# Yuki-11/CSBSR

Hardware: AMD Instinct MI355X
Metric: training imgs/s (448->1792 x4, PSPNet) (higher is better)
Workload: dtype fp16 storage / fp32 accumulate (detector forward: split fp16 hi+lo); 1 GPU; CSBSR KBPN x4 + PSPNet, beta=0.3, joint phase (iter 40000), per-GPU batch 8, LR 448x448 -> HR 1792x1792, fwd+loss+bwd+Adam; batch resident in HBM (H2D outside `value`, timed beside it as with_h2d_inside_step); full-size synthetic crack images degraded on the device; global_batch=8, micro_batch=8, parallelism=dp1

## Files before the change

csbsr_amd/_lib.py:

```python
import ctypes as C
import os
from collections import namedtuple

import torch

_HERE = os.path.dirname(os.path.abspath(__file__))
LIB_PATH = os.environ.get("CSBSR_LIB") or os.path.join(_HERE, "libcsbsr_hip.so")

ACT_NONE, ACT_RELU, ACT_LRELU, ACT_PRELU, ACT_SIGMOID = 0, 1, 2, 3, 4
RES_NONE, RES_ADD, RES_SUB, RES_MUL, RES_FMA = 0, 1, 2, 3, 4
STAT_NONE, STAT_BN, STAT_SAMPLE_SUM = 0, 1, 2

i32, i64, f32, vp = C.c_int32, C.c_int64, C.c_float, C.c_void_p


class Seg(C.Structure):
    _fields_ = [("ptr", vp), ("sn", i64), ("sy", i64), ("sx", i64), ("c", i32), ("creal", i32)]


class ConvDesc(C.Structure):
    _fields_ = [("inp", Seg * 2), ("N", i32), ("H", i32), ("W", i32), ("OH", i32), ("OW", i32),
                ("transposed", i32), ("KH", i32), ("KW", i32), ("stride", i32), ("pad", i32), ("dil", i32),
                ("wt", vp), ("cout", i32), ("coutp", i32),
                ("out16", vp), ("o_sn", i64), ("o_sy", i64), ("o_sx", i64),
# ... 73 lines not shown
    "csbsr_maxpool3x3s2_bwd_split": (i32, [vp, i64, i64, vp, i64, i64, vp, vp, i32, i32, i32, i32, vp]),
    "csbsr_adaptive_avgpool_fwd_split": (i32, [vp, i64, i64, vp, i64, i64, i32, i32, i32, i32, i32, i32, vp]),
    "csbsr_sum_act_split": (i32, [i64, i32, i32, vp, vp, vp, vp, i64, i64, i32, vp]),
    "csbsr_weighted_pool_fwd_split": (i32, [vp, i64, i64, vp, vp, i32, i64, i32, vp]),
    "csbsr_bilinear_fwd_split": (i32, [vp, i64, i64, vp, i64, i64, i32, i32, i32, i32, i32, i32, i32, vp, vp]),
    "csbsr_unpack_wgrad": (i32, [vp, vp] + [i32] * 9 + [f32, i32, i32, vp]),
    "csbsr_wgrad_splits": (i32, [i32, i32, i64]),
    "csbsr_wgrad_splits_desc": (i32, [vp]),
    "csbsr_epilogue_backward": (i32, [C.POINTER(EpiBwdDesc), vp]),
    "csbsr_set_reduction_scratch": (i32, [vp, i64]),
    "csbsr_axpby": (i32, [i64, i32, vp, i64, f32, vp, i64, f32, vp, i64, vp]),
    "csbsr_fill_f16": (i32, [vp, i64, i32, i64, f32, vp]),
    "csbsr_sum_act": (i32, [i64, i32, i32, vp, vp, vp, i64, i32, vp]),
    "csbsr_weighted_pool_fwd": (i32, [vp, i64, vp, vp, i32, i64, i32, vp]),
    "csbsr_weighted_pool_bwd": (i32, [vp, i64, vp, vp, vp, i64, vp, i32, i64, i32, vp]),
    "csbsr_nchw32_to_nhwc16": (i32, [vp, vp, i32, i32, i32, i32, i32, i64, vp, vp, vp]),
    "csbsr_nhwc16_to_nchw32": (i32, [vp, i64, vp, i32, i32, i32, i32, f32, f32, vp]),
    "csbsr_plane_reduce": (i32, [vp, vp, i32, i64, vp, vp]),
    "csbsr_channel_mean_sub": (i32, [vp, i64, i64, i64, i32, i32, i32, i32, i32, vp, vp]),
    "csbsr_thin_tp_backward_slabs": (i32, [i32, i32]),
    "csbsr_conv_thin_dact_eligible": (i32, [vp]),
    "csbsr_conv_split_fused_eligible": (i32, [C.POINTER(ConvDesc)]),
    "csbsr_thin_tp_backward": (i32, [vp, i64, i64, i64, vp, i64, i64, i64, vp, i32, i32, i32, i32, vp, i32, i32, i32, vp, i64, i64, i64, vp, vp, vp]),
    "csbsr_round_weights": (i32, [vp, vp, vp, i32, i32, i32, i32, i32, vp]),
    "csbsr_dc_bias": (i32, [vp, i32, i32, vp, i64, i32, vp, i64, i32, vp, i32, vp, vp]),
    "csbsr_instnorm_bwd": (i32, [vp, i64, vp, vp, vp, vp, i32, i32, i32, i64, vp, vp]),
    "csbsr_border_class_fill": (i32, [vp, vp, i64, i32, i32, i32, i32, vp]),
    "csbsr_border_class_fill_masked": (i32, [vp, vp, i64, vp, i64, C.c_float, i32, i32, i32, i32, vp]),
    "csbsr_border_class_sums": (i32, [vp, i64, vp, i32, i32, i32, i32, vp]),
    "csbsr_border_class_sums_prelu": (i32, [vp, i64, vp, i64, vp, vp, i32, i32, i32, i32, vp]),
    "csbsr_ring_class_sums": (i32, [vp, i64, vp, i32, i32, i32, i32, vp]),
    "csbsr_bn_finalize": (i32, [vp, i64, i32, i32, f32, f32, vp, vp, vp, vp, vp]),
    "csbsr_bn_apply": (i32, [C.POINTER(BnDesc), vp]),
    "csbsr_bn_backward": (i32, [C.POINTER(BnDesc), vp]),
    "csbsr_maxpool3x3s2_fwd": (i32, [vp, vp, i32, i32, i32, i32, vp]),
    "csbsr_maxpool3x3s2_bwd": (i32, [vp, vp, vp, vp, i32, i32, i32, i32, vp]),
    "csbsr_adaptive_avgpool_fwd": (i32, [vp, i64, vp, i32, i32, i32, i32, i32, i32, vp]),
    "csbsr_adaptive_avgpool_bwd": (i32, [vp, vp, i64, i32, i32, i32, i32, i32, i32, i32, vp]),
    "csbsr_bilinear_fwd": (i32, [vp, i64, vp, i64, i32, i32, i32, i32, i32, i32, i32, vp, vp]),
    "csbsr_bilinear_bwd": (i32, [vp, i64, vp, i64, i32, i32, i32, i32, i32, i32, i32, i32, vp, vp]),
    "csbsr_bilinear32_fwd": (i32, [vp, vp, i32, i32, i32, i32, i32, i32, vp]),
    "csbsr_bilinear32_bwd": (i32, [vp, vp, i32, i32, i32, i32, i32, i32, vp]),
    "csbsr_bicubic_up_add": (i32, [vp, vp, i32, i32, i32, i32, vp]),
    "csbsr_aa_bicubic_up": (i32, [vp, vp, i32, i32, i32, i32, i32, i32, vp]),
    "csbsr_aa_bicubic_down_fwd": (i32, [vp, vp, i32, i32, i32, i32, i32, vp]),
    "csbsr_aa_bicubic_down_bwd": (i32, [vp, vp, i32, i32, i32, i32, i32, i32, vp]),
    "csbsr_area_down_fwd": (i32, [vp, vp, i32, i32, i32, i32, vp]),
    "csbsr_area_down_bwd": (i32, [vp, vp, i32, i32, i32, i32, i32, vp]),
    "csbsr_blur_fwd": (i32, [vp, vp, i32, i32, i32, i32, i32, i32, vp, vp, vp, i64, vp]),
    "csbsr_blur_bwd_input": (i32, [vp, vp, vp, i32, i32, i32, i32, i32, i32, i32, vp]),
    "csbsr_blur_bwd_kernel": (i32, [vp, vp, vp, i32, i32, i32, i32, i32, i32, vp]),
    "csbsr_sdf": (i32, [vp, vp, vp, i32, i32, i32, vp]),
# ... 98 lines not shown
```

csbsr_amd/csrc/elementwise.hip:

```cpp
#include <cstdlib>
#include "common.h"

static inline int grid_for(long work, int block = 256, int cap = 8192) {
  long b = (work + block - 1) / block;
  if (b < 1) b = 1;
  return (int)(b > cap ? cap : b);
}
#define ST(s) reinterpret_cast<hipStream_t>(s)

__device__ __forceinline__ void ld_split(const half_t* p, long lo, float (&v)[8]) {
  const h8 a = *reinterpret_cast<const h8*>(p);
#pragma unroll
  for (int e = 0; e < 8; ++e) v[e] = (float)a[e];
  if (lo) {
    const h8 b = *reinterpret_cast<const h8*>(p + lo);
#pragma unroll
    for (int e = 0; e < 8; ++e) v[e] += (float)b[e];
  }
}
__device__ __forceinline__ void st_split(half_t* p, long lo, const float (&v)[8]) {
  h8 a, b;
#pragma unroll
  for (int e = 0; e < 8; ++e) { a[e] = (half_t)v[e]; b[e] = (half_t)(v[e] - (float)a[e]); }
  *reinterpret_cast<h8*>(p) = a;
// ... 1746 lines not shown
}
__global__ void bcs_edges_finish_kernel(const float* part, float* sums, int N, int c) {
  const int i = blockIdx.x * blockDim.x + threadIdx.x;
  if (i >= N * 4 * 3 * c) return;
  const int ch = i % c; int r = i / c;
  const int k = r % 3; r /= 3;
  const int edge = r % 4; const int n = r / 4;
  if (edge >= 2 && k > 0) return;
  const int base_cls = edge == 0 ? 8 : (edge == 1 ? 4 : (edge == 2 ? 2 : 1));
  const int cls = base_cls + (k == 1 ? 2 : (k == 2 ? 1 : 0));
  float t = 0.f;
  for (int seg = 0; seg < BCS_SEG; ++seg) t += part[((((long)n * 4 + edge) * BCS_SEG + seg) * 3 + k) * c + ch];
  sums[((long)n * 16 + cls) * c + ch] += t;
}
__global__ void bcs_fixup_kernel(float* sums, int N, int c) {
  const int i = blockIdx.x * blockDim.x + threadIdx.x;
  if (i >= N * c) return;
  const int n = i / c, ch = i % c;
  float* s_ = sums + (long)n * 16 * c + ch;
  float border = 0.f;
  for (int k = 1; k < 16; ++k) border += s_[(long)k * c];
  s_[0] -= border;
}
static int border_class_sums_impl(const void* x, int64_t ld, float* sums, int32_t N, int32_t H, int32_t W, int32_t c, const void* t, int64_t t_ld,
                                  float* negdot, csbsr_stream_t s) {
  CSBSR_CHECK(x && sums && c % 8 == 0, "border_class_sums: bad args");
  CSBSR_CHECK(!t || (negdot && H >= 3 && W >= 3 && (long)H * W >= 1024), "border_class_sums_prelu: maps of >= 1024 pixels, negdot required");
  if (H >= 3 && W >= 3 && (long)H * W >= 1024) {
    const long hw = (long)H * W;
    int chunks = (int)((hw + 511) / 512);
    if (chunks > 2048) chunks = 2048;
    const long n_tot = (long)N * chunks * c, n_edge = (long)N * 4 * BCS_SEG * 3 * c;
    float* part = csbsr_red_scratch(n_tot + n_edge + (t ? n_tot : 0));
    CSBSR_NEED_SCRATCH(part, "border_class_sums");
    if (t) {
      float* part2 = part + n_tot + n_edge;
      hipLaunchKernelGGL(bcs_total_kernel<true>, dim3(N * chunks), dim3(256), 0, ST(s), (const half_t*)x, (long)ld, sums, hw, c / 8, chunks, part,
                         (const half_t*)t, (long)t_ld, part2);
      if (csbsr_sum_partials_batched(part2, chunks, c, c, negdot, N, (long)c, ST(s))) return 1;
    } else {
      hipLaunchKernelGGL(bcs_total_kernel<false>, dim3(N * chunks), dim3(256), 0, ST(s), (const half_t*)x, (long)ld, sums, hw, c / 8, chunks, part,
                         (const half_t*)nullptr, 0l, (float*)nullptr);
    }
    if (csbsr_sum_partials_batched(part, chunks, c, c, sums, N, 16l * c, ST(s))) return 1;
    float* epart = part + n_tot;
    hipLaunchKernelGGL(bcs_edges_kernel, dim3(N * 4 * ((c / 8 + 31) / 32) * BCS_SEG), dim3(256), 0, ST(s), (const half_t*)x, (long)ld, epart, H, W, c / 8);
    hipLaunchKernelGGL(bcs_edges_finish_kernel, dim3((N * 12 * c + 255) / 256), dim3(256), 0, ST(s), (const float*)epart, sums, N, c);
    hipLaunchKernelGGL(bcs_fixup_kernel, dim3((N * c + 255) / 256), dim3(256), 0, ST(s), sums, N, c);
    CSBSR_LAUNCH_CHECK("csbsr_border_class_sums");
    return 0;
  }
  hipLaunchKernelGGL(border_class_sums_small_kernel, dim3(N), dim3(256), 0, ST(s), (const half_t*)x, (long)ld, sums, H, W, c / 8);
  CSBSR_LAUNCH_CHECK("csbsr_border_class_sums");
  return 0;
}
extern "C" int csbsr_border_class_sums(const void* x, int64_t ld, float* sums, int32_t N, int32_t H, int32_t W, int32_t c, csbsr_stream_t s) {
  return border_class_sums_impl(x, ld, sums, N, H, W, c, nullptr, 0, nullptr, s);
}
extern "C" int csbsr_border_class_sums_prelu(const void* x, int64_t ld, const void* t, int64_t t_ld, float* sums, float* negdot, int32_t N, int32_t H,
                                             int32_t W, int32_t c, csbsr_stream_t s) {
  CSBSR_CHECK(t && negdot, "border_class_sums_prelu: null pointer");
  return border_class_sums_impl(x, ld, sums, N, H, W, c, t, t_ld, negdot, s);
}

__global__ __launch_bounds__(256) void rcs_lines_kernel(const half_t* x, long ld, float* part, int H, int W, int c8) {
  __shared__ float sbin[8][5][32][8];
  const int groups = (c8 + 31) / 32;
  int b = blockIdx.x;
  const int seg = b % BCS_SEG; b /= BCS_SEG;
  const int g = b % groups; b /= groups;
  const int line = b % 8; const int n = b / 8;
  const int cl = threadIdx.x & 31, pl = threadIdx.x >> 5;
  const int cc = g * 32 + cl;
  const bool is_row = line < 4;
  const int coord = (line & 3) < 2 ? (line & 3) : ((is_row ? H : W) - 4 + (line & 3));
  const int lo = is_row ? 0 : 2, hi = is_row ? W : H - 2;
  float a[5][8];
#pragma unroll
  for (int k = 0; k < 5; ++k)
#pragma unroll
// ... 70 lines not shown
```

csbsr_amd/modeling/kbpn.py:

```python
import ctypes as C

import os

import torch
import torch.nn.functional as F

from .. import _lib as L
from ..engine import FM, Conv, ShuffleConv, grad_acc, pad8, _ptr
from .blocks import act_bwd, sft_bwd
from .shapes import CONV_SETTING

A_NONE, A_RELU, A_LRELU, A_PRELU, A_SIG = L.ACT_NONE, L.ACT_RELU, L.ACT_LRELU, L.ACT_PRELU, L.ACT_SIGMOID


class _Stage:
    pass


def border_tap_mask():
    m = torch.ones(4, 3)
    m[2, 0] = m[3, 0] = 0.0
    m[1, 2] = m[3, 2] = 0.0
    return m


def ring_tap_classes():
    r = torch.zeros(5, 3, 4)
    r[0, 1, 2] = r[0, 2, 0] = 1.0
    r[1, 0, 2] = r[1, 1, 0] = r[1, 2, 0] = 1.0
    r[2, :, 0] = 1.0
    r[3, 0, 0] = r[3, 1, 0] = r[3, 2, 1] = 1.0
    r[4, 0, 0] = r[4, 1, 1] = 1.0
# ... 84 lines not shown
                for c_ in (o.sc0, o.sc1, o.sh0, o.sh1):
                    c_.winograd = True
            self.stages.append(o)
        self.output_conv = block(f"{prefix}.output_conv", 3, 1, 1, A_NONE)
        for c in self.layers:
            c.dc_comp = ".kernel_predictor." not in c.name
        eye = torch.eye(kc).reshape(kc, 1, cfg.ksize, cfg.ksize)
        up = F.interpolate(eye, size=(self.K, self.K), mode="bicubic", align_corners=False) if cfg.ksize != self.K else eye
        self.U = up.reshape(kc, self.kk).t().contiguous().to(eng.device)
        self.zero_pad = bool(getattr(cfg, "zero_pad_kernel", False))
        self.pad_dropout = True
        self._pad_replay, self.pad_taken = None, []
        pz = (self.K - cfg.ksize) // 2
        self.Z = F.pad(eye, (pz, pz, pz, pz)).reshape(kc, self.kk).t().contiguous().to(eng.device)
        if self.zero_pad:
            for st_i, o in enumerate(self.stages):
                pd = f"{prefix}.back_projection_stages.{st_i}.kb.kernel_predictor.pad_descriminator"
                o.pad_disc = [(P[f"{pd}.{i}.weight"], P[f"{pd}.{i}.bias"]) for i in (0, 3, 6)]
        self.kc = kc
        self.saved = None
        self.training_mode = True
        self._gather = {}
        self.gather = os.environ.get("CSBSR_GATHER_DCH", "1") != "0"
        self.Mtap = border_tap_mask().to(eng.device)
        self.Rtap = ring_tap_classes().to(eng.device)

    def set_phase(self, it):
        c = self.cfg
        sr_pre = c.sr_pretrain[0] <= it < c.sr_pretrain[1]
        k_pre = c.kernel_pretrain[0] <= it < c.kernel_pretrain[1]
        self.use_predictor = not sr_pre
        for l in self.layers:
            n = l.name
            is_kernel = ("kernel_predictor" in n) or (".predictor." in n)
            if sr_pre:
                l.frozen = is_kernel
            elif k_pre:
                l.frozen = not is_kernel
            else:
                l.frozen = False

    def invalidate(self):
        for l in self.layers:
            l.invalidate()
        self._gather = {}

# ... 330 lines not shown
                else:
                    c.bwd_input(dz, out=dinit, accumulate=True)
        d = dinit
        for i in (3, 2, 1, 0):
            c = self.feat[i]
            act_bwd(c, d, feats[i + 1])
            self._wg(c, d, feats[i])
            if i > 0:
                d = c.bwd_input(d)
        self.saved = None
        e.join_wgrad()
        if stage_done is not None:
            stage_done(0)

    def _kernel_predictor_bwd(self, st, q, dk2, dsr_t, H, W):
        e = self.eng
        a, kctx, c1, c2 = q["kp"]
        if len(a) == 1:
            a = list(a)
            for c in st.fe_sr:
                a.append(c.fwd(a[-1]))
        B = dk2.shape[0]
        d49 = torch.einsum("bk,bkc->bc", dk2, q["kp_map"]) / float(H * W)
        g = self._bcast_grad(d49, H, W)
        cat2, cat1, cat0 = st.fe_cat[2], st.fe_cat[1], st.fe_cat[0]
        msk = lambda conv, out: (out, 0.0 if conv.act == A_RELU else conv.slope)
        self._wg(cat2, g, c2)
        dc2 = self._fold_const_dgrad(cat2, d49, msk(cat1, c2), H, W)
        self._wg(cat1, dc2, c1)
        dc1 = cat1.bwd_input(dc2, mask=msk(cat0, c1))
        del dc2
        if not cat0.frozen:
            cat0.bwd_weights(dc1, a[-1], split_override=(cat0.split[0], 0))
        da = cat0.bwd_input(dc1, seg=0, mask=msk(st.fe_sr[4], a[5]))
        dkin = self._kernel_branch_bwd(st, dc1, kctx, H, W)
        del dc1
        for i in (4, 3, 2, 1, 0):
            c = st.fe_sr[i]
            self._wg(c, da, a[i])
            if i > 0:
                da = c.bwd_input(da, mask=msk(st.fe_sr[i - 1], a[i]))
            else:
                c.bwd_input(da, out32=dsr_t, accumulate=True)
        return dk2 + dkin

    def _kernel_branch_fwd(self, st, kvec, H, W):
        e = self.eng
        assert H >= 5 and W >= 5, "two-ring classes need a map of at least 5 x 5"
        k0, k1, cat0 = st.fe_k[0], st.fe_k[1], st.fe_cat[0]
        with torch.enable_grad():
            kv = kvec.detach().to(torch.float32).requires_grad_(True)
            w0, w1, wc = (c.w.detach().requires_grad_(not c.frozen) for c in (k0, k1, cat0))
            cbv = kernel_branch_table(kv, w0, w1, wc[:, cat0.split[0]:, 0, 0], self.Mtap, self.Rtap, _act_fn(k0), _act_fn(k1))
        cb = e.f32(kvec.shape[0], 25, pad8(cat0.cout))
        cb[:, :, :cat0.cout] = cbv.detach().reshape(-1, 25, cat0.cout)
        return cb, (cbv, kv, (w0, w1, wc))

    def _kernel_branch_bwd(self, st, dc1, kctx, H, W):
        e = self.eng
        cbv, kv, ws = kctx
        cat0 = st.fe_cat[0]
        B = dc1.N
        sums = e.f32(B, 25, dc1.cp)
        L.call("csbsr_ring_class_sums", _ptr(dc1.t), dc1.ld, _ptr(sums), B, H, W, dc1.cp, e.stream)
        leaves = [kv] + [w for w in ws if w.requires_grad]
        grads = torch.autograd.grad(cbv, leaves, sums[:, :, :cat0.cout].reshape(B, 5, 5, cat0.cout))
        gi = iter(grads[1:])
        for conv, w in zip((st.fe_k[0], st.fe_k[1], cat0), ws):
            if w.requires_grad:
                g = next(gi)
                if conv is cat0:
                    c0 = cat0.split[0]
                    grad_acc(conv.w)[:, c0:].add_(g[:, c0:])
                else:
                    grad_acc(conv.w).add_(g)
        return grads[0]

    def _fold_const_dgrad(self, conv, gvec, mask, H, W):
        e = self.eng
        B = gvec.shape[0]
        w16 = conv.w.to(torch.float16).float()
        g16 = gvec.to(torch.float16).float()
        T = torch.einsum("no,ocyx->ncyx", g16, w16)
        mf = self.Mtap.flip(1)
        V = torch.einsum("ncyx,ay,bx->nabc", T, mf, mf)
        cp = pad8(conv.cin)
        Vp = e.f32(B, 16, cp)
        Vp[:, :, :conv.cin] = V.reshape(B, 16, conv.cin)
        out = e.new(B, H, W, conv.cin)
        mfm, mslope = mask
        assert mfm.cp == cp and (mfm.H, mfm.W) == (H, W) and not mfm.bcast
        L.call("csbsr_border_class_fill_masked", _ptr(Vp), _ptr(out.t), out.ld, _ptr(mfm.t), mfm.ld, float(mslope), B, H, W, cp, e.stream)
        return out
```

csbsr_amd/utils/kernel_names.py:

```python
import re

_CONV = {0: "conv_igemm_kernel<32,4,1>", 1: "conv_igemm_kernel<64,2,2>", 2: "conv_igemm_kernel<128,2,2>", 5: "conv_thin_cout_kernel",
         6: "conv_thin_cin_kernel", 11: "conv_thin_tp_kernel", 13: "conv_thin_cin2_kernel", 15: "conv_thin_sc_kernel", 16: "conv_thin_tpd_kernel",
         10: "conv_x3_kernel<3>", 12: "conv_x3_kernel<2>", 17: "conv_x3_kernel<3,1024>", 18: "conv_x3_kernel<2,1024>"}
HEAD1_FWD, HEAD1_BWD_INPUT = 21, 22
_GLDS = {3: (128, 2, 2, 1), 4: (256, 4, 3, 1), 7: (256, 4, 2, 2), 14: (128, 2, 2, 0)}
_WGRAD = {0: "conv_wgrad_kernel<128,128,2,2>", 1: "conv_wgrad_kernel<128,256,2,4>", 2: "conv_wgrad_kernel<64,128,2,2>",
          3: "conv_wgrad_kernel<32,128,1,4>", 4: "conv_wgrad_thin_kernel", 5: "conv_wgrad_glds_kernel<128,128>",
          6: "conv_wgrad_glds_kernel<128,256>", 7: "conv_wgrad_glds_kernel<256,256>", 8: "conv_wgrad_hr_kernel",
          9: "conv_wgrad_glds_kernel<128,512>"}


def conv_row(kid):
    base, var = kid & 255, kid >> 8
    if base in _GLDS:
        bm, nwm, ns, ct = _GLDS[base]
        return f"conv_igemm_glds_kernel<{bm},{nwm},{ns},{ct},FS={var & 1},GK={(var >> 1) & 1}>"
    if base == 9:
        return f"conv_tp_kernel<res={var & 1},acc={(var >> 1) & 1},mask={(var >> 2) & 1},sums={(var >> 3) & 1}>"
    if base == 8:
        return (f"conv_hr_kernel<{7 if var & 1 else 4},stat={(var >> 4) & 1},taps={1 if var & 2 else 9},nct={2 if var & 4 else 1},"
                f"mask={(var >> 3) & 1},cb={(var >> 5) & 1}>")
    if base == 10 and var & 1:
        return "conv_x3_kernel<3,2048>"
# ... 32 lines not shown
        return "conv_wgrad_glds_kernel<%s,%s>" % m.groups()
    m = re.search(r"conv_wgrad_kernel<(\d+), (\d+), (\d+), (\d+)", name) or re.search(r"conv_wgrad_kernelILi(\d+)ELi(\d+)ELi(\d+)ELi(\d+)E", name)
    if m:
        return "conv_wgrad_kernel<%s,%s,%s,%s>" % m.groups()
    m = (re.search(r"conv_hr_kernelILi(\d+)ELb(\d)ELi(\d+)ELi(\d+)ELb(\d)ELb(\d)E", name)
         or re.search(r"conv_hr_kernel<(\d+), (\w+), (\d+), (\d+), (\w+), (\w+)>", name))
    if m:
        g = m.groups()
        return "conv_hr_kernel<%s,stat=%s,taps=%s,nct=%s,mask=%s,cb=%s>" % (g[0], _b(g[1]), g[2], g[3], _b(g[4]), _b(g[5]))
    m = re.search(r"conv_tp_kernelILi\d+ELb(\d)ELb(\d)ELb(\d)ELb(\d)E", name) or re.search(r"conv_tp_kernel<\d+, (\w+), (\w+), (\w+), (\w+)>", name)
    if m:
        return "conv_tp_kernel<res=%s,acc=%s,mask=%s,sums=%s>" % tuple(_b(x) for x in m.groups())
    m = (re.search(r"conv_x3n_kernelILb(\d)ELb(\d)ELb(\d)ELb(\d)E", name)
         or re.search(r"conv_x3n_kernel<(\w+), (\w+), (\w+), (\w+)>", name))
    if m:
        return "conv_x3n_kernel<%s,%s%s%s>" % (_b(m.group(1)), _b(m.group(2)), ",wide" if _b(m.group(3)) == "1" else "",
                                               ",lean" if _b(m.group(4)) == "1" else "")
    m = re.search(r"conv_x3w_kernelILi(\d)E", name) or re.search(r"conv_x3w_kernel<(\d)>", name)
    if m:
        return "conv_x3w_kernel<%s>" % m.group(1)
    m = re.search(r"conv_x3_kernelILi(\d)ELi(\d+)E", name) or re.search(r"conv_x3_kernel<(\d), (\d+)>", name)
    if m:
        return "conv_x3_kernel<%s>" % m.group(1) if m.group(2) == "0" else "conv_x3_kernel<%s,%s>" % m.groups()
    for k in ("conv_wgrad_hr_kernel", "conv_wgrad_thin_kernel", "conv_wgrad_kernel", "conv_thin_cout_kernel", "conv_thin_cin2_kernel", "conv_thin_cin_kernel",
              "conv_thin_tpd_kernel", "conv_thin_tp_kernel", "conv_thin_sc_kernel", "thin_tp_bwd_kernel", "epilogue_bwd_kernel", "unpack_wgrad_kernel",
              "head1_fwd_kernel", "head1_bwd_input_kernel", "bn_bwd_apply_kernel", "bn_bwd_reduce_kernel", "bn_apply_kernel", "channel_mean_sub_kernel", "round_weights_kernel"):
        if k in name:
            return k
    return name[:60]
```

include/csbsr_hip.h:

```cpp
#ifndef CSBSR_HIP_H
#define CSBSR_HIP_H
#include <stdint.h>
#ifdef __cplusplus
extern "C" {
#endif

typedef void* csbsr_stream_t;

int csbsr_version(void);
const char* csbsr_last_error(void);

enum { CSBSR_ACT_NONE = 0, CSBSR_ACT_RELU = 1, CSBSR_ACT_LRELU = 2, CSBSR_ACT_PRELU = 3, CSBSR_ACT_SIGMOID = 4 };
enum { CSBSR_RES_NONE = 0, CSBSR_RES_ADD = 1, CSBSR_RES_SUB = 2, CSBSR_RES_MUL = 3, CSBSR_RES_FMA = 4 };
enum { CSBSR_STAT_NONE = 0, CSBSR_STAT_BN = 1 ,
       CSBSR_STAT_SAMPLE_SUM = 2  };

typedef struct {
  const void* ptr;
  int64_t sn, sy, sx;
  int32_t c;
  int32_t creal;
} csbsr_seg_t;

typedef struct {
// ... 171 lines not shown
int csbsr_weighted_pool_bwd(const void* x, int64_t x_ld, const float* w, const float* dout, void* dx, int64_t dx_ld, float* dw,
                            int32_t N, int64_t hw, int32_t c, csbsr_stream_t s);

int csbsr_nchw32_to_nhwc16(const float* src, void* dst, int32_t N, int32_t C, int32_t H, int32_t W, int32_t cp,
                           int64_t dst_ld, const float* mean, const float* invstd, csbsr_stream_t s);
int csbsr_nhwc16_to_nchw32(const void* src, int64_t src_ld, float* dst, int32_t N, int32_t C, int32_t H, int32_t W,
                           float alpha, float beta, csbsr_stream_t s);
int csbsr_plane_reduce(const float* a, const float* b, int32_t planes, int64_t hw, float* out, csbsr_stream_t s);
int csbsr_channel_mean_sub(const void* x, int64_t sn, int64_t sy, int64_t sx, int32_t N, int32_t H, int32_t W, int32_t cp,
                           int32_t step, float* out, csbsr_stream_t s);
int csbsr_round_weights(const float* w, float* wq, float* S, int32_t D0, int32_t D1, int32_t KH, int32_t KW, int32_t mode, csbsr_stream_t s);
int csbsr_dc_bias(const float* S, int32_t cout, int32_t cin, const float* m0, int64_t m0_ld, int32_t c0, const float* m1, int64_t m1_ld,
                  int32_t c1, const float* bias, int32_t N, float* out, csbsr_stream_t s);
int csbsr_instnorm_bwd(const void* dy, int64_t dy_ld, const float* x, const float* mean, const float* invstd,
                       float* dx, int32_t accumulate, int32_t N, int32_t C, int64_t hw, float* red,
                       csbsr_stream_t s);

int csbsr_border_class_fill(const float* V, void* out, int64_t ld, int32_t N, int32_t H, int32_t W, int32_t c,
                            csbsr_stream_t s);
int csbsr_border_class_fill_masked(const float* V, void* out, int64_t ld, const void* mask, int64_t mask_ld, float mask_slope, int32_t N,
                                   int32_t H, int32_t W, int32_t c, csbsr_stream_t s);
int csbsr_border_class_sums(const void* x, int64_t ld, float* sums, int32_t N, int32_t H, int32_t W, int32_t c,
                            csbsr_stream_t s);
int csbsr_border_class_sums_prelu(const void* x, int64_t ld, const void* t, int64_t t_ld, float* sums, float* negdot, int32_t N, int32_t H,
                                  int32_t W, int32_t c, csbsr_stream_t s);
int csbsr_ring_class_sums(const void* x, int64_t ld, float* sums, int32_t N, int32_t H, int32_t W, int32_t c,
                          csbsr_stream_t s);

int csbsr_bn_finalize(const float* stat, int64_t count, int32_t c, int32_t cstride, float eps, float momentum,
                      float* mean, float* invstd, float* running_mean, float* running_var, csbsr_stream_t s);
typedef struct {
  int64_t npix, hw;
  int32_t c, creal;
  const void* x; int64_t x_ld;
  const float *mean, *invstd, *gamma, *beta;
  const void* res; int64_t res_ld;
  int32_t act; int32_t _pad;
  const float* prelu;
  const float* drop;
  void* y; int64_t y_ld;
  const void* dy; int64_t dy_ld;
  float* red;
  float* dprelu;
  void* dx; int64_t dx_ld;
  void* dres; int64_t dres_ld; int32_t dres_accumulate; int32_t _pad1;
  float *dgamma, *dbeta;
// ... 63 lines not shown
                         float* out_f32, uint8_t* out_u8, csbsr_stream_t s);
int csbsr_stitch_tiles_u8(const float* patches, int32_t N, int32_t C, int32_t PH, int32_t PW, const int32_t* tiles, const int64_t* offsets,
                          const int32_t* dims, int32_t clip, float* out_f32, uint8_t* out_u8, csbsr_stream_t s);
int csbsr_threshold_planes_u8(const float* pred, const float* thresholds, int32_t N, int64_t hw, int32_t S, uint8_t* out, csbsr_stream_t s);
int csbsr_iou_sweep(const float* pred, const float* mask, const float* thresholds, int32_t N, int64_t hw, int32_t T, float smooth,
                    uint32_t* hist, float* iou, float* inter, float* uni, csbsr_stream_t s);
int csbsr_psnr_ssim(const float* a, const float* b, int32_t N, int32_t C, int32_t H, int32_t W, float* sums, float* psnr, float* ssim,
                    csbsr_stream_t s);

int csbsr_surface_prepare(const float* pred, const float* mask, const float* thresholds, int32_t H, int32_t W, int32_t T, uint8_t* lvl,
                          uint8_t* gt, int32_t* counts, int32_t* rowflag, uint16_t* gcol, int32_t* dgt, csbsr_stream_t s);
int csbsr_surface_gather(const uint8_t* lvl, const uint8_t* gt, const int32_t* dgt, const int32_t* rowflag, int32_t H, int32_t W, int32_t j0,
                         int32_t nj, uint16_t* gcol, const int32_t* tab_off, const int32_t* tab_cap, int32_t* tab_keys, uint32_t* tab_cnt,
                         int32_t max_cap, int32_t* rows, int32_t max_rows, int32_t* meta, csbsr_stream_t s);

int csbsr_pr_sweep(const float* pred, const float* mask, const float* thresholds, int32_t N, int32_t H, int32_t W, int32_t T, int32_t tol2,
                   uint32_t* hist, int32_t* counts, csbsr_stream_t s);

int32_t csbsr_thin_tp_backward_slabs(int32_t N, int32_t h);
int csbsr_thin_tp_backward(const void* dout, int64_t d_sn, int64_t d_sy, int64_t d_sx, const void* x, int64_t x_sn, int64_t x_sy,
                           int64_t x_sx, const void* wt_packed, int32_t cin, int32_t cout, int32_t stride, int32_t pad,
                           const float* prelu, int32_t N, int32_t h, int32_t w, void* dpre, int64_t p_sn, int64_t p_sy, int64_t p_sx,
                           float* slabs, float* dprelu_part, csbsr_stream_t s);
int32_t csbsr_conv_split_fused_eligible(const csbsr_conv_desc_t* d);
int32_t csbsr_conv_thin_dact_eligible(const csbsr_conv_desc_t* d);
#ifdef __cplusplus
}
#endif
#endif
```

Before: 8.203 imgs/s.

## Fuse 1x1 conv dgrad+wgrad pair kernel and fold constant-grad wgrad into masked fill

```diff
diff --git a/csbsr_amd/_lib.py b/csbsr_amd/_lib.py
--- a/csbsr_amd/_lib.py
+++ b/csbsr_amd/_lib.py
@@ -119,12 +119,15 @@
     "csbsr_conv_thin_dact_eligible": (i32, [vp]),
     "csbsr_conv_split_fused_eligible": (i32, [C.POINTER(ConvDesc)]),
     "csbsr_thin_tp_backward": (i32, [vp, i64, i64, i64, vp, i64, i64, i64, vp, i32, i32, i32, i32, vp, i32, i32, i32, vp, i64, i64, i64, vp, vp, vp]),
+    "csbsr_conv_pair1x1_slabs": (i32, [i32, i32, i32, vp]),
+    "csbsr_conv_pair1x1_backward": (i32, [vp, i64, i64, i64, vp, i64, i64, i64, vp, f32, i32, i32, i32, vp, i64, i64, i64, vp, vp]),
     "csbsr_round_weights": (i32, [vp, vp, vp, i32, i32, i32, i32, i32, vp]),
     "csbsr_dc_bias": (i32, [vp, i32, i32, vp, i64, i32, vp, i64, i32, vp, i32, vp, vp]),
     "csbsr_instnorm_bwd": (i32, [vp, i64, vp, vp, vp, vp, i32, i32, i32, i64, vp, vp]),
     "csbsr_border_class_fill": (i32, [vp, vp, i64, i32, i32, i32, i32, vp]),
     "csbsr_border_class_fill_masked": (i32, [vp, vp, i64, vp, i64, C.c_float, i32, i32, i32, i32, vp]),
     "csbsr_border_class_sums": (i32, [vp, i64, vp, i32, i32, i32, i32, vp]),
+    "csbsr_border_class_fill_masked_sums": (i32, [vp, vp, i64, vp, i64, C.c_float, vp, i32, i32, i32, i32, vp]),
     "csbsr_border_class_sums_prelu": (i32, [vp, i64, vp, i64, vp, vp, i32, i32, i32, i32, vp]),
     "csbsr_ring_class_sums": (i32, [vp, i64, vp, i32, i32, i32, i32, vp]),
     "csbsr_bn_finalize": (i32, [vp, i64, i32, i32, f32, f32, vp, vp, vp, vp, vp]),
diff --git a/csbsr_amd/csrc/conv_pair.hip b/csbsr_amd/csrc/conv_pair.hip
--- /dev/null
+++ b/csbsr_amd/csrc/conv_pair.hip
@@ -0,0 +1,240 @@
+#include "common.h"
+#include "conv_wgrad.h"
+
+#define PR_TH 8
+#define PR_TW 32
+#define PR_NBUF 3
+
+struct PairK {
+  const half_t* a; long a_sn, a_sy, a_sx;
+  const half_t* b; long b_sn, b_sy, b_sx;
+  int N, H, W;
+  const half_t* wt;
+  half_t* out; long o_sn, o_sy, o_sx;
+  float aslope, mask_slope;
+  float* g; long slab_stride;
+  unsigned tiles_x, tiles_y;
+};
+
+constexpr int PR_PA = 80, PR_PB = 112;
+constexpr int PR_NPA = PR_TH * PR_TW * PR_PA / 4096, PR_NPB = PR_TH * PR_TW * PR_PB / 4096, PR_NPW = PR_NPA + PR_NPB;
+constexpr int PR_ABYTES = PR_NPA * 4096, PR_BUF = PR_NPW * 4096;
+constexpr int PR_SMEM = PR_NBUF * PR_BUF + 256;
+static_assert(PR_TH * PR_TW * PR_PA % 4096 == 0 && PR_TH * PR_TW * PR_PB % 4096 == 0, "whole pieces");
+static_assert(PR_SMEM <= 160 * 1024, "LDS budget");
+
+typedef int pr_v4i __attribute__((ext_vector_type(4)));
+static __device__ __forceinline__ void pr_dma16(pr_v4i rs, int voff, unsigned lds_addr) {
+  unsigned keep;
+  asm volatile("s_mov_b32 %0, m0\n\ts_mov_b32 m0, %3\n\ts_nop 0\n\tbuffer_load_dwordx4 %1, %2, 0 offen lds\n\ts_mov_b32 m0, %0"
+               : "=&s"(keep) : "v"(voff), "s"(rs), "s"(lds_addr));
+}
+static __device__ __forceinline__ pr_v4i pr_make_rs(const half_t* base) {
+  const unsigned long a = reinterpret_cast<unsigned long>(base);
+  pr_v4i r;
+  r[0] = __builtin_amdgcn_readfirstlane((int)(unsigned)a);
+  r[1] = __builtin_amdgcn_readfirstlane((int)((unsigned)(a >> 32) & 0xffffu));
+  r[2] = 0x7fffffff;
+  r[3] = 0x00020000;
+  return r;
+}
+
+__global__ __launch_bounds__(256) void conv_pair1x1_kernel(const PairK p) {
+#if defined(__HIP_DEVICE_COMPILE__)
+  constexpr int PA = PR_PA, PB = PR_PB, NPA = PR_NPA, NPW = PR_NPW, ABYTES = PR_ABYTES, BUF = PR_BUF, NBUF = PR_NBUF;
+  constexpr int R = 4;
+  extern __shared__ __attribute__((aligned(16))) char smem[];
+  const int tid = threadIdx.x, lane = tid & 63;
+  const int wid = __builtin_amdgcn_readfirstlane(tid >> 6);
+  const int pix = lane & 31, hi = lane >> 5;
+  const int ctl = wid >> 1, row0 = (wid & 1) * R;
+  const int bb = wid & 1, part = wid >> 1;
+  const unsigned per_img = p.tiles_x * p.tiles_y, total = per_img * (unsigned)p.N, gsub = gridDim.x;
+
+  h8 wf[2];
+#pragma unroll
+  for (int ks = 0; ks < 2; ++ks) wf[ks] = *reinterpret_cast<const h8*>(p.wt + ((size_t)(ctl * 2 + ks) * 64 + lane) * 8);
+
+  int voff[NPW], py0[NPW], px0[NPW];
+#pragma unroll
+  for (int i = 0; i < NPW; ++i) {
+    const bool isa = i < NPA;
+    const int g = (wid + 4 * (isa ? i : i - NPA)) * 64 + lane, slots = isa ? 5 : 7, px = g / slots, c = g - px * slots;
+    const int ty = px / PR_TW, tx = px - ty * PR_TW;
+    voff[i] = 2 * (int)(isa ? ty * p.a_sy + tx * p.a_sx + c * 8 : ty * p.b_sy + tx * p.b_sx + c * 8);
+    py0[i] = (isa && c >= 4) ? 0x40000000 : ty;
+    px0[i] = tx;
+  }
+  auto tile_at = [&](unsigned vb, int& n, int& y0, int& x0) {
+    if (vb >= total) vb -= ((vb - total) / gsub + 1) * gsub;
+    const unsigned lt = xcd_remap(vb, total);
+    n = lt / per_img;
+    const unsigned r_ = lt - n * per_img;
+    y0 = (r_ / p.tiles_x) * PR_TH; x0 = (r_ % p.tiles_x) * PR_TW;
+  };
+  const unsigned lds0 = (unsigned)(unsigned long)((__attribute__((address_space(3))) char*)smem) + (unsigned)wid * 1024u;
+  auto issue_piece = [&](pr_v4i rsa, pr_v4i rsb, int y0, int x0, int j, int buf) __attribute__((always_inline)) {
+    const bool ok = (unsigned)(py0[j] + y0) < (unsigned)p.H && (unsigned)(px0[j] + x0) < (unsigned)p.W;
+    if (j < NPA) pr_dma16(rsa, ok ? voff[j] : -1, lds0 + (unsigned)(buf * BUF + 4 * j * 1024));
+    else pr_dma16(rsb, ok ? voff[j] : -1, lds0 + (unsigned)(buf * BUF + ABYTES + 4 * (j - NPA) * 1024));
+  };
+  auto src_a = [&](int n, int y0, int x0) { return p.a + n * p.a_sn + (long)y0 * p.a_sy + (long)x0 * p.a_sx; };
+  auto src_b = [&](int n, int y0, int x0) { return p.b + n * p.b_sn + (long)y0 * p.b_sy + (long)x0 * p.b_sx; };
+
+  const int li = lane & 15;
+  const int rsub = (lane >> 5) * 8 + (li >> 2);
+  const int unit = (lane >> 4) & 1;
+  const int aoff = rsub * PA + unit * 32 + (li & 3) * 8 + (part * R) * PR_TW * PA;
+  const int boff = ABYTES + rsub * PB + (bb * 2 + unit) * 32 + (li & 3) * 8 + (part * R) * PR_TW * PB;
+  auto tr8 = [&](const char* q, int rowbytes) __attribute__((always_inline)) {
+    const fp16x4 r0 = __builtin_amdgcn_ds_read_tr16_b64_v4f16((__attribute__((address_space(3))) fp16x4*)(q));
+    const fp16x4 r1 = __builtin_amdgcn_ds_read_tr16_b64_v4f16((__attribute__((address_space(3))) fp16x4*)(q + 4 * rowbytes));
+    h8 v;
+    v[0] = r0[0]; v[1] = r0[1]; v[2] = r0[2]; v[3] = r0[3]; v[4] = r1[0]; v[5] = r1[1]; v[6] = r1[2]; v[7] = r1[3];
+    return v;
+  };
+  const int doff = (row0 * PR_TW + pix) * PA + hi * 16;
+  const int moff = ABYTES + (row0 * PR_TW + pix) * PB + (ctl * 32 + 8 * hi) * 2;
+
+  f16v gacc;
+#pragma unroll
+  for (int r = 0; r < 16; ++r) gacc[r] = 0.f;
+
+  const unsigned j0 = blockIdx.x;
+  if (j0 < total) {
+#pragma unroll
+    for (int k = 0; k < NBUF - 1; ++k) {
+      int n, y0, x0;
+      tile_at(j0 + k * gsub, n, y0, x0);
+      const pr_v4i rsa = pr_make_rs(src_a(n, y0, x0)), rsb = pr_make_rs(src_b(n, y0, x0));
+#pragma unroll
+      for (int j = 0; j < NPW; ++j) issue_piece(rsa, rsb, y0, x0, j, k);
+    }
+    int buf = 0;
+    for (unsigned vb = j0; vb < total; vb += gsub) {
+      int n, y0, x0, nn, y0n, x0n;
+      tile_at(vb, n, y0, x0);
+      tile_at(vb + (NBUF - 1) * gsub, nn, y0n, x0n);
+      const pr_v4i rsa = pr_make_rs(src_a(nn, y0n, x0n)), rsb = pr_make_rs(src_b(nn, y0n, x0n));
+      const int bfill = buf == 0 ? NBUF - 1 : buf - 1;
+      asm volatile("s_waitcnt vmcnt(%0)" ::"n"((NBUF - 2) * NPW) : "memory");
+      __builtin_amdgcn_s_barrier();
+      asm volatile("" ::: "memory");
+      const char* tb = smem + buf * BUF;
+
+      f16v acc[R];
+#pragma unroll
+      for (int q = 0; q < R; ++q)
+#pragma unroll
+        for (int r = 0; r < 16; ++r) acc[q][r] = 0.f;
+      h8 bfr[R];
+#pragma unroll
+      for (int q = 0; q < R; ++q) bfr[q] = *reinterpret_cast<const h8*>(tb + doff + q * PR_TW * PA);
+#pragma unroll
+      for (int ks = 0; ks < 2; ++ks)
+#pragma unroll
+        for (int q = 0; q < R; ++q) {
+          acc[q] = __builtin_amdgcn_mfma_f32_32x32x16_f16(wf[ks], bfr[q], acc[q], 0, 0, 0);
+          if (ks == 0) bfr[q] = *reinterpret_cast<const h8*>(tb + doff + q * PR_TW * PA + 32);
+          issue_piece(rsa, rsb, y0n, x0n, ks * R + q, bfill);
+        }
+#pragma unroll
+      for (int r = 0; r < R; ++r)
+#pragma unroll
+        for (int h = 0; h < 2; ++h) {
+          const h8 af = tr8(tb + aoff + (r * PR_TW + h * 16) * PA, PA);
+          const h8 bf = tr8(tb + boff + (r * PR_TW + h * 16) * PB, PB);
+          gacc = __builtin_amdgcn_mfma_f32_32x32x16_f16(af, bf, gacc, 0, 0, 0);
+          const int j = 2 * R + r * 2 + h;
+          if (j < NPW) issue_piece(rsa, rsb, y0n, x0n, j, bfill);
+        }
+#pragma unroll
+      for (int q = 0; q < R; ++q) {
+        const int oy = y0 + row0 + q, ox = x0 + pix;
+        const bool live = oy < p.H && ox < p.W;
+#pragma unroll
+        for (int pair = 0; pair < 2; ++pair) {
+          const h8 mk = *reinterpret_cast<const h8*>(tb + moff + q * PR_TW * PB + 32 * pair);
+          float v[8];
+#pragma unroll
+          for (int j = 0; j < 4; ++j) {
+            const unsigned a = __float_as_uint(acc[q][8 * pair + j]), b = __float_as_uint(acc[q][8 * pair + 4 + j]);
+            auto r = __builtin_amdgcn_permlane32_swap(a, b, false, false);
+            v[j] = __uint_as_float(r[0]);
+            v[4 + j] = __uint_as_float(r[1]);
+          }
+          const int co = ctl * 32 + 16 * pair + 8 * hi;
+#pragma unroll
+          for (int e = 0; e < 8; ++e) v[e] = fmaxf(v[e], v[e] * p.aslope);
+#pragma unroll
+          for (int e = 0; e < 8; ++e) v[e] *= ((float)mk[e] > 0.f ? 1.f : p.mask_slope);
+          if (live && co < 56) {
+            h8 hv;
+#pragma unroll
+            for (int e = 0; e < 8; ++e) hv[e] = (half_t)v[e];
+            *reinterpret_cast<h8*>(p.out + n * p.o_sn + oy * p.o_sy + ox * p.o_sx + co) = hv;
+          }
+        }
+      }
+      buf = buf + 1 == NBUF ? 0 : buf + 1;
+    }
+  }
+
+  asm volatile("s_waitcnt vmcnt(0)" ::: "memory");
+  __syncthreads();
+  float* red = reinterpret_cast<float*>(smem);
+  if (part == 1) {
+#pragma unroll
+    for (int r = 0; r < 16; ++r) red[(bb * 16 + r) * 64 + lane] = gacc[r];
+  }
+  __syncthreads();
+  if (part == 0) {
+    float* slab = p.g + (size_t)blockIdx.x * p.slab_stride;
+    const int b = bb * 32 + (lane & 31);
+#pragma unroll
+    for (int r = 0; r < 16; ++r) {
+      const float v = gacc[r] + red[(bb * 16 + r) * 64 + lane];
+      const int row = (r & 3) + 8 * (r >> 2) + 4 * (lane >> 5);
+      if (b < 56) slab[(size_t)row * 56 + b] = v;
+    }
+  }
+#endif
+}
+
+static bool pair_geometry_ok(int64_t a_sy, int64_t b_sy, int64_t a_sx, int64_t b_sx, int64_t o_sx) {
+  return a_sy < (1l << 31) / 32 && b_sy < (1l << 31) / 32 && a_sx >= 32 && b_sx >= 56 && o_sx >= 56 && a_sx % 8 == 0 && b_sx % 8 == 0 && o_sx % 8 == 0;
+}
+
+static unsigned pair_grid(int32_t N, int32_t H, int32_t W, hipStream_t st) {
+  const unsigned total = (unsigned)N * (unsigned)((H + PR_TH - 1) / PR_TH) * (unsigned)((W + PR_TW - 1) / PR_TW);
+  unsigned g = (unsigned)csbsr_cu_budget(st);
+  if (g > total) g = total;
+  return (g + 7) / 8 * 8;
+}
+
+extern "C" int32_t csbsr_conv_pair1x1_slabs(int32_t N, int32_t H, int32_t W, csbsr_stream_t s) {
+  if (N < 1 || H < 1 || W < 1) return 0;
+  return (int32_t)pair_grid(N, H, W, reinterpret_cast<hipStream_t>(s));
+}
+
+extern "C" int csbsr_conv_pair1x1_backward(const void* dpre, int64_t a_sn, int64_t a_sy, int64_t a_sx, const void* x, int64_t b_sn, int64_t b_sy,
+                                           int64_t b_sx, const void* wt_packed, float mask_slope, int32_t N, int32_t H, int32_t W, void* din,
+                                           int64_t o_sn, int64_t o_sy, int64_t o_sx, float* slabs, csbsr_stream_t s) {
+  CSBSR_CHECK(dpre && x && wt_packed && din && slabs && N >= 1 && H >= 1 && W >= 1, "conv_pair1x1: bad args");
+  CSBSR_CHECK(pair_geometry_ok(a_sy, b_sy, a_sx, b_sx, o_sx), "conv_pair1x1: strides (row stride too large for 32-bit piece offsets, or pixels not 16-byte chunks)");
+  hipStream_t st = reinterpret_cast<hipStream_t>(s);
+  PairK k;
+  k.a = reinterpret_cast<const half_t*>(dpre); k.a_sn = a_sn; k.a_sy = a_sy; k.a_sx = a_sx;
+  k.b = reinterpret_cast<const half_t*>(x); k.b_sn = b_sn; k.b_sy = b_sy; k.b_sx = b_sx;
+  k.N = N; k.H = H; k.W = W;
+  k.wt = reinterpret_cast<const half_t*>(wt_packed);
+  k.out = reinterpret_cast<half_t*>(din); k.o_sn = o_sn; k.o_sy = o_sy; k.o_sx = o_sx;
+  k.aslope = 1.f; k.mask_slope = mask_slope;
+  k.g = slabs; k.slab_stride = 32l * 56;
+  k.tiles_x = (unsigned)((W + PR_TW - 1) / PR_TW); k.tiles_y = (unsigned)((H + PR_TH - 1) / PR_TH);
+  static LdsAttrOnce attr;
+  if (int e = csbsr_lds_attr(attr, reinterpret_cast<const void*>(conv_pair1x1_kernel), PR_SMEM, "conv_pair1x1")) return e;
+  hipLaunchKernelGGL(conv_pair1x1_kernel, dim3(pair_grid(N, H, W, st)), dim3(256), PR_SMEM, st, k);
+  CSBSR_LAUNCH_CHECK("csbsr_conv_pair1x1_backward");
+  return 0;
+}
diff --git a/csbsr_amd/csrc/elementwise.hip b/csbsr_amd/csrc/elementwise.hip
--- a/csbsr_amd/csrc/elementwise.hip
+++ b/csbsr_amd/csrc/elementwise.hip
@@ -1792,6 +1792,11 @@
   for (int k = 1; k < 16; ++k) border += s_[(long)k * c];
   s_[0] -= border;
 }
+static void bcs_border_classes(const void* x, int64_t ld, float* sums, int32_t N, int32_t H, int32_t W, int32_t c, float* epart, csbsr_stream_t s) {
+  hipLaunchKernelGGL(bcs_edges_kernel, dim3(N * 4 * ((c / 8 + 31) / 32) * BCS_SEG), dim3(256), 0, ST(s), (const half_t*)x, (long)ld, epart, H, W, c / 8);
+  hipLaunchKernelGGL(bcs_edges_finish_kernel, dim3((N * 12 * c + 255) / 256), dim3(256), 0, ST(s), (const float*)epart, sums, N, c);
+  hipLaunchKernelGGL(bcs_fixup_kernel, dim3((N * c + 255) / 256), dim3(256), 0, ST(s), sums, N, c);
+}
 static int border_class_sums_impl(const void* x, int64_t ld, float* sums, int32_t N, int32_t H, int32_t W, int32_t c, const void* t, int64_t t_ld,
                                   float* negdot, csbsr_stream_t s) {
   CSBSR_CHECK(x && sums && c % 8 == 0, "border_class_sums: bad args");
@@ -1813,10 +1818,7 @@
                          (const half_t*)nullptr, 0l, (float*)nullptr);
     }
     if (csbsr_sum_partials_batched(part, chunks, c, c, sums, N, 16l * c, ST(s))) return 1;
-    float* epart = part + n_tot;
-    hipLaunchKernelGGL(bcs_edges_kernel, dim3(N * 4 * ((c / 8 + 31) / 32) * BCS_SEG), dim3(256), 0, ST(s), (const half_t*)x, (long)ld, epart, H, W, c / 8);
-    hipLaunchKernelGGL(bcs_edges_finish_kernel, dim3((N * 12 * c + 255) / 256), dim3(256), 0, ST(s), (const float*)epart, sums, N, c);
-    hipLaunchKernelGGL(bcs_fixup_kernel, dim3((N * c + 255) / 256), dim3(256), 0, ST(s), sums, N, c);
+    bcs_border_classes(x, ld, sums, N, H, W, c, part + n_tot, s);
     CSBSR_LAUNCH_CHECK("csbsr_border_class_sums");
     return 0;
   }
@@ -1826,6 +1828,69 @@
 }
 extern "C" int csbsr_border_class_sums(const void* x, int64_t ld, float* sums, int32_t N, int32_t H, int32_t W, int32_t c, csbsr_stream_t s) {
   return border_class_sums_impl(x, ld, sums, N, H, W, c, nullptr, 0, nullptr, s);
+}
+
+__global__ __launch_bounds__(256) void bcs_fill_total_kernel(const float* V, half_t* out, long ld, const half_t* mask, long mld, float mslope, int H, int W,
+                                                             int c8, int chunks, float* part) {
+  __shared__ float sred[256][8];
+  const long hw = (long)H * W;
+  const int n = blockIdx.x / chunks, chunk = blockIdx.x % chunks;
+  const int cpb = c8 < 256 ? c8 : 256, ppb = 256 / cpb;
+  const int ch = threadIdx.x % cpb, pl = threadIdx.x / cpb;
+  const long per = (hw + chunks - 1) / chunks;
+  const long beg = chunk * per, end = beg + per < hw ? beg + per : hw;
+  for (int cbase = 0; cbase < c8; cbase += cpb) {
+    const int cc = cbase + ch;
+    float a[8];
+#pragma unroll
+    for (int e = 0; e < 8; ++e) a[e] = 0.f;
+    if (cc < c8 && pl < ppb)
+      for (long px = beg + pl; px < end; px += ppb) {
+        const h8 m = *reinterpret_cast<const h8*>(mask + ((long)n * hw + px) * mld + cc * 8);
+        const int y = (int)(px / W), x = (int)(px - (long)y * W);
+        const int cls = (y == 0) * 8 + (y == H - 1) * 4 + (x == 0) * 2 + (x == W - 1);
+        const float* v = V + ((long)n * 16 + cls) * c8 * 8 + cc * 8;
+        h8 o;
+#pragma unroll
+        for (int e = 0; e < 8; ++e) {
+          a[e] += (float)m[e];
+          o[e] = (half_t)(v[e] * ((float)m[e] > 0.f ? 1.f : mslope));
+        }
+        *reinterpret_cast<h8*>(out + ((long)n * hw + px) * ld + cc * 8) = o;
+      }
+#pragma unroll
+    for (int e = 0; e < 8; ++e) sred[threadIdx.x][e] = a[e];
+    __syncthreads();
+    if (threadIdx.x < cpb && cbase + threadIdx.x < c8) {
+#pragma unroll
+      for (int e = 0; e < 8; ++e) {
+        float s_ = 0.f;
+        for (int q = 0; q < ppb; ++q) s_ += sred[q * cpb + threadIdx.x][e];
+        part[(long)blockIdx.x * c8 * 8 + (cbase + threadIdx.x) * 8 + e] = s_;
+      }
+    }
+    __syncthreads();
+  }
+}
+extern "C" int csbsr_border_class_fill_masked_sums(const float* V, void* out, int64_t ld, const void* mask, int64_t mask_ld, float mask_slope, float* sums,
+                                                   int32_t N, int32_t H, int32_t W, int32_t c, csbsr_stream_t s) {
+  CSBSR_CHECK(V && out && mask && sums && c % 8 == 0, "border_class_fill_masked_sums: bad args");
+  if (!(H >= 3 && W >= 3 && (long)H * W >= 1024)) {
+    if (int e = csbsr_border_class_fill_masked(V, out, ld, mask, mask_ld, mask_slope, N, H, W, c, s)) return e;
+    return csbsr_border_class_sums(mask, mask_ld, sums, N, H, W, c, s);
+  }
+  const long hw = (long)H * W;
+  int chunks = (int)((hw + 511) / 512);
+  if (chunks > 2048) chunks = 2048;
+  const long n_tot = (long)N * chunks * c, n_edge = (long)N * 4 * BCS_SEG * 3 * c;
+  float* part = csbsr_red_scratch(n_tot + n_edge);
+  CSBSR_NEED_SCRATCH(part, "border_class_fill_masked_sums");
+  hipLaunchKernelGGL(bcs_fill_total_kernel, dim3(N * chunks), dim3(256), 0, ST(s), V, (half_t*)out, (long)ld, (const half_t*)mask, (long)mask_ld, mask_slope,
+                     H, W, c / 8, chunks, part);
+  if (csbsr_sum_partials_batched(part, chunks, c, c, sums, N, 16l * c, ST(s))) return 1;
+  bcs_border_classes(mask, mask_ld, sums, N, H, W, c, part + n_tot, s);
+  CSBSR_LAUNCH_CHECK("csbsr_border_class_fill_masked_sums");
+  return 0;
 }
 extern "C" int csbsr_border_class_sums_prelu(const void* x, int64_t ld, const void* t, int64_t t_ld, float* sums, float* negdot, int32_t N, int32_t H,
                                              int32_t W, int32_t c, csbsr_stream_t s) {
diff --git a/csbsr_amd/modeling/kbpn.py b/csbsr_amd/modeling/kbpn.py
--- a/csbsr_amd/modeling/kbpn.py
+++ b/csbsr_amd/modeling/kbpn.py
@@ -8,6 +8,7 @@
 from .. import _lib as L
 from ..engine import FM, Conv, ShuffleConv, grad_acc, pad8, _ptr
 from .blocks import act_bwd, sft_bwd
+from .kp_bwd import const_wgrad_ok, fold_const_wgrad, pair1x1_backward, pair1x1_ok
 from .shapes import CONV_SETTING
 
 A_NONE, A_RELU, A_LRELU, A_PRELU, A_SIG = L.ACT_NONE, L.ACT_RELU, L.ACT_LRELU, L.ACT_PRELU, L.ACT_SIGMOID
@@ -138,6 +139,7 @@
         self.training_mode = True
         self._gather = {}
         self.gather = os.environ.get("CSBSR_GATHER_DCH", "1") != "0"
+        self.kp_pairs = int(os.environ.get("CSBSR_KP_BWD_PAIRS", "3"))
         self.Mtap = border_tap_mask().to(eng.device)
         self.Rtap = ring_tap_classes().to(eng.device)
 
@@ -514,21 +516,33 @@
                 a.append(c.fwd(a[-1]))
         B = dk2.shape[0]
         d49 = torch.einsum("bk,bkc->bc", dk2, q["kp_map"]) / float(H * W)
-        g = self._bcast_grad(d49, H, W)
         cat2, cat1, cat0 = st.fe_cat[2], st.fe_cat[1], st.fe_cat[0]
         msk = lambda conv, out: (out, 0.0 if conv.act == A_RELU else conv.slope)
-        self._wg(cat2, g, c2)
-        dc2 = self._fold_const_dgrad(cat2, d49, msk(cat1, c2), H, W)
+        fold, pairs = int(self.kp_pairs) & 1, int(self.kp_pairs) & 2
+        if fold and not cat2.frozen and const_wgrad_ok(cat2):
+            sums = e.f32(B, 16, c2.cp)
+            dc2 = self._fold_const_dgrad(cat2, d49, msk(cat1, c2), H, W, sums=sums)
+            fold_const_wgrad(cat2, d49, sums, self.Mtap)
+        else:
+            self._wg(cat2, self._bcast_grad(d49, H, W), c2)
+            dc2 = self._fold_const_dgrad(cat2, d49, msk(cat1, c2), H, W)
         self._wg(cat1, dc2, c1)
         dc1 = cat1.bwd_input(dc2, mask=msk(cat0, c1))
         del dc2
-        if not cat0.frozen:
-            cat0.bwd_weights(dc1, a[-1], split_override=(cat0.split[0], 0))
-        da = cat0.bwd_input(dc1, seg=0, mask=msk(st.fe_sr[4], a[5]))
+        mslope = msk(st.fe_sr[4], a[5])[1]
+        if pairs and not cat0.frozen and pair1x1_ok(cat0, dc1, a[5]):
+            da = pair1x1_backward(cat0, dc1, a[5], mslope)
+        else:
+            if not cat0.frozen:
+                cat0.bwd_weights(dc1, a[-1], split_override=(cat0.split[0], 0))
+            da = cat0.bwd_input(dc1, seg=0, mask=msk(st.fe_sr[4], a[5]))
         dkin = self._kernel_branch_bwd(st, dc1, kctx, H, W)
         del dc1
         for i in (4, 3, 2, 1, 0):
             c = st.fe_sr[i]
+            if i > 0 and pairs and not c.frozen and pair1x1_ok(c, da, a[i]):
+                da = pair1x1_backward(c, da, a[i], msk(st.fe_sr[i - 1], a[i])[1])
+                continue
             self._wg(c, da, a[i])
             if i > 0:
                 da = c.bwd_input(da, mask=msk(st.fe_sr[i - 1], a[i]))
@@ -568,7 +582,7 @@
                     grad_acc(conv.w).add_(g)
         return grads[0]
 
-    def _fold_const_dgrad(self, conv, gvec, mask, H, W):
+    def _fold_const_dgrad(self, conv, gvec, mask, H, W, sums=None):
         e = self.eng
         B = gvec.shape[0]
         w16 = conv.w.to(torch.float16).float()
@@ -582,5 +596,9 @@
         out = e.new(B, H, W, conv.cin)
         mfm, mslope = mask
         assert mfm.cp == cp and (mfm.H, mfm.W) == (H, W) and not mfm.bcast
-        L.call("csbsr_border_class_fill_masked", _ptr(Vp), _ptr(out.t), out.ld, _ptr(mfm.t), mfm.ld, float(mslope), B, H, W, cp, e.stream)
+        if sums is not None:
+            L.call("csbsr_border_class_fill_masked_sums", _ptr(Vp), _ptr(out.t), out.ld, _ptr(mfm.t), mfm.ld, float(mslope), _ptr(sums), B, H, W, cp,
+                   e.stream)
+        else:
+            L.call("csbsr_border_class_fill_masked", _ptr(Vp), _ptr(out.t), out.ld, _ptr(mfm.t), mfm.ld, float(mslope), B, H, W, cp, e.stream)
         return out
diff --git a/csbsr_amd/modeling/kp_bwd.py b/csbsr_amd/modeling/kp_bwd.py
--- /dev/null
+++ b/csbsr_amd/modeling/kp_bwd.py
@@ -0,0 +1,45 @@
+import torch
+
+from .. import _lib as L
+from ..engine import _ptr, grad_acc, pad8
+
+
+def fold_const_wgrad(conv, gvec, sums, mtap):
+    B, cin = gvec.shape[0], conv.cin
+    g16 = gvec.to(torch.float16).float()
+    mf = mtap.flip(1)
+    S = torch.einsum("nabc,ay,bx->ncyx", sums[:, :, :cin].reshape(B, 4, 4, cin), mf, mf)
+    grad_acc(conv.w).add_(torch.einsum("no,ncyx->ocyx", g16, S))
+
+
+def const_wgrad_ok(conv):
+    return (not conv.transposed and conv.k == 3 and conv.stride == 1 and conv.pad == 1 and conv.dil == 1 and conv.split[1] == 0
+            and conv.b is None)
+
+
+def pair1x1_ok(conv, dpre, x, seg0=None):
+    c0 = conv.split[0] if seg0 is None else seg0
+    return (conv.eng.use_hr and not conv.transposed and conv.k == 1 and conv.stride == 1 and conv.pad == 0 and conv.b is None
+            and not conv.hp_dgrad and conv.cout == 32 and dpre.cp == 32 and pad8(c0) == 56 and x.cp == 56 and x.c == c0
+            and c0 <= conv.w.shape[1] and not (dpre.bcast or x.bcast or dpre.lo or x.lo)
+            and (dpre.N, dpre.H, dpre.W) == (x.N, x.H, x.W))
+
+
+def pair1x1_backward(conv, dpre, x, mask_slope, seg0=None):
+    eng = conv.eng
+    c0 = conv.split[0] if seg0 is None else seg0
+    assert pair1x1_ok(conv, dpre, x, seg0)
+    key = ("hr", 1, 0)
+    wt = conv._packed.get(key)
+    if wt is None:
+        wt = conv._pack_new(key, conv._wq(), "csbsr_packed_weight_elems_hr", (1, conv.cout, c0),
+                            "csbsr_pack_weights_hr", (1, 1, *conv.w.shape[:2], conv.cout, c0, 0, 0))
+    N, H, W = dpre.N, dpre.H, dpre.W
+    out = eng.new(N, H, W, c0)
+    ns = int(L.load().csbsr_conv_pair1x1_slabs(N, H, W, eng.stream))
+    slabs = eng.workspace(ns * 32 * 56)
+    L.call("csbsr_conv_pair1x1_backward", _ptr(dpre.t), *dpre.strides(), _ptr(x.t), *x.strides(), _ptr(wt), float(mask_slope), N, H, W,
+           _ptr(out.t), *out.strides(), _ptr(slabs), eng.stream)
+    L.call("csbsr_unpack_wgrad", _ptr(slabs), _ptr(grad_acc(conv.w)), 32, 1, 1, c0, 0, conv.w.shape[0], conv.w.shape[1], 0, 0, 1.0, ns, 32,
+           eng.stream)
+    return out
diff --git a/csbsr_amd/utils/kernel_names.py b/csbsr_amd/utils/kernel_names.py
--- a/csbsr_amd/utils/kernel_names.py
+++ b/csbsr_amd/utils/kernel_names.py
@@ -78,7 +78,7 @@
     m = re.search(r"conv_x3_kernelILi(\d)ELi(\d+)E", name) or re.search(r"conv_x3_kernel<(\d), (\d+)>", name)
     if m:
         return "conv_x3_kernel<%s>" % m.group(1) if m.group(2) == "0" else "conv_x3_kernel<%s,%s>" % m.groups()
-    for k in ("conv_wgrad_hr_kernel", "conv_wgrad_thin_kernel", "conv_wgrad_kernel", "conv_thin_cout_kernel", "conv_thin_cin2_kernel", "conv_thin_cin_kernel",
+    for k in ("conv_pair1x1_kernel", "bcs_fill_total_kernel", "conv_wgrad_hr_kernel", "conv_wgrad_thin_kernel", "conv_wgrad_kernel", "conv_thin_cout_kernel", "conv_thin_cin2_kernel", "conv_thin_cin_kernel",
               "conv_thin_tpd_kernel", "conv_thin_tp_kernel", "conv_thin_sc_kernel", "thin_tp_bwd_kernel", "epilogue_bwd_kernel", "unpack_wgrad_kernel",
               "head1_fwd_kernel", "head1_bwd_input_kernel", "bn_bwd_apply_kernel", "bn_bwd_reduce_kernel", "bn_apply_kernel", "channel_mean_sub_kernel", "round_weights_kernel"):
         if k in name:
diff --git a/include/csbsr_hip.h b/include/csbsr_hip.h
--- a/include/csbsr_hip.h
+++ b/include/csbsr_hip.h
@@ -217,6 +217,8 @@
                                    int32_t H, int32_t W, int32_t c, csbsr_stream_t s);
 int csbsr_border_class_sums(const void* x, int64_t ld, float* sums, int32_t N, int32_t H, int32_t W, int32_t c,
                             csbsr_stream_t s);
+int csbsr_border_class_fill_masked_sums(const float* V, void* out, int64_t ld, const void* mask, int64_t mask_ld, float mask_slope,
+                                        float* sums, int32_t N, int32_t H, int32_t W, int32_t c, csbsr_stream_t s);
 int csbsr_border_class_sums_prelu(const void* x, int64_t ld, const void* t, int64_t t_ld, float* sums, float* negdot, int32_t N, int32_t H,
                                   int32_t W, int32_t c, csbsr_stream_t s);
 int csbsr_ring_class_sums(const void* x, int64_t ld, float* sums, int32_t N, int32_t H, int32_t W, int32_t c,
@@ -326,6 +328,10 @@
                            int64_t x_sx, const void* wt_packed, int32_t cin, int32_t cout, int32_t stride, int32_t pad,
                            const float* prelu, int32_t N, int32_t h, int32_t w, void* dpre, int64_t p_sn, int64_t p_sy, int64_t p_sx,
                            float* slabs, float* dprelu_part, csbsr_stream_t s);
+int32_t csbsr_conv_pair1x1_slabs(int32_t N, int32_t H, int32_t W, csbsr_stream_t s);
+int csbsr_conv_pair1x1_backward(const void* dpre, int64_t a_sn, int64_t a_sy, int64_t a_sx, const void* x, int64_t b_sn, int64_t b_sy,
+                                int64_t b_sx, const void* wt_packed, float mask_slope, int32_t N, int32_t H, int32_t W, void* din,
+                                int64_t o_sn, int64_t o_sy, int64_t o_sx, float* slabs, csbsr_stream_t s);
 int32_t csbsr_conv_split_fused_eligible(const csbsr_conv_desc_t* d);
 int32_t csbsr_conv_thin_dact_eligible(const csbsr_conv_desc_t* d);
 #ifdef __cplusplus
```

After: 8.320 imgs/s (median of 6 runs). 1.4% higher.
